# aynik/carta1

Measured on AMD Instinct MI355X. Metric: atrac1_stereo_frames_per_s_encode, higher is better.
Workload: dtype f32+f64

## Files before the change

### carta1_amd/csrc/c1_k_spec.hip

```cpp
#include "c1_device.h"

namespace {

constexpr int kR2 = 840;
constexpr int kMemFloats = kR2 + 576;
constexpr int kIn2 = 1;
struct alignas(16) SpecLds {
  alignas(16) float mem[kMemFloats];
  alignas(16) float d1[48];
  alignas(16) float d2[48];
  alignas(16) float pre2[76];
  alignas(4) uint8_t sfi[64];
  uint32_t geo[3][64];
};
constexpr int kSpecWaves = 4;
constexpr int kSpecTabBase = (int)offsetof(C1DevTables, win32);
constexpr int kSpecTabFloats = ((int)offsetof(C1DevTables, r2d) + (int)sizeof(((C1DevTables *)nullptr)->r2d) - kSpecTabBase) / 4;
static_assert(offsetof(C1DevTables, pre32_64) > offsetof(C1DevTables, win32) && offsetof(C1DevTables, r2d) > offsetof(C1DevTables, r4c) &&
              offsetof(C1DevTables, norm32) == offsetof(C1DevTables, r2d) + sizeof(((C1DevTables *)nullptr)->r2d), "win32 .. r2d are one contiguous block");
static_assert(kSpecWaves * sizeof(SpecLds) + kSpecTabFloats * 4 + 27 * 16 <= 32768, "speculative analysis: 5 workgroups of 4 waves per CU");
constexpr int kE2 = 0, kH2 = 288, kE0 = kR2, kH0 = kR2 + 160, kE1 = kR2 + 288, kH1 = kR2 + 448;

__device__ __forceinline__ int w1_phys(int v) { return __mul24(12, v >> 3) + (v & 7); }

template <int D, int NP>
__device__ __forceinline__ void qmf_core_f32(const v2f (&W)[NP], TablesPtr T, float (&lo)[D], float (&hi)[D]) {
  v2f tp[26];
#pragma unroll
  for (int j = 0; j < 26; j++) tp[j] = *reinterpret_cast<const __attribute__((address_space(4))) v2f *>(T->tap_pair[j]);
  const float e12 = T->tap32[12];
#pragma unroll
  for (int d = 0; d < D; d++) {
    v2f p1 = W[d + 23] * tp[0];
#pragma unroll
    for (int j = 1; j <= 10; j++) p1 = pk_fma(W[d + 23 - j], tp[j], p1);
    v2f p2 = W[d] * tp[23];
#pragma unroll
    for (int j = 22; j >= 13; j--) p2 = pk_fma(W[d + 23 - j], tp[j], p2);
    p1 = pk_fma(W[d + 12], tp[24], p1);
    p2 = pk_fma(W[d + 11], tp[25], p2);
    const v2f sum = p1 + p2;
    const float ev = __builtin_fmaf(e12, W[d + 11].y, sum.y);
    const float od = __builtin_fmaf(e12, W[d + 12].x, sum.x);
    lo[d] = ev + od;
    hi[d] = ev - od;
  }
}

struct SpecBase {
  int ia0, ic0;
  int q2;
  int ib, id;
  int pt0;
  int za, zb, zc, zd;
  int g;
  int e0, e1;
  int po0;
  bool band0, band2, use_lo, use_hi;
};
__device__ __forceinline__ SpecBase spec_base(int lane) {
  SpecBase B;
  const int band = lane < 16 ? 0 : (lane < 32 ? 1 : 2);
  const int g = lane - (band == 0 ? 0 : (band == 1 ? 16 : 32));
  const int n4 = band == 2 ? 128 : 64, q = n4 / 4;
  const int r = bitrev(g, band == 2 ? 5 : 4);
  const int in_base = band == 0 ? kR2 : (band == 1 ? kR2 + 256 : kIn2);
  const int tab_base = band == 2 ? (int)offsetof(C1DevTables, pre32_512) : (int)offsetof(C1DevTables, pre32_256);
  B.ia0 = in_base + 3 * n4 - 1 - 2 * r;
  B.ic0 = in_base + n4 + 2 * r;
  B.q2 = 2 * q;
  B.use_lo = r < 8;
  B.use_hi = r >= q - 8;
  B.ib = B.use_lo ? in_base + 3 * n4 + 2 * r : in_base + 2 * r + 2 * q;
  B.id = B.use_lo ? in_base + n4 - 1 - 2 * r : in_base + 14 * q - 1 - 2 * r;
  B.pt0 = tab_base + 8 * r;
  const int pbase = band == 0 ? 0 : (band == 1 ? 64 : 128);
  B.za = zslot(pbase + 4 * g);
  B.zb = zslot(pbase + 16 * (g >> 2) + (g & 3));
  B.zc = zslot(pbase + 64 * (g >> 4) + (g & 15));
  B.zd = zslot(128 + (g & 31));
  B.g = g;
  const int cbase = band == 0 ? 0 : (band == 1 ? 128 : 256), n2 = 2 * n4;
  B.e0 = cbase + 2 * g;
  B.e1 = cbase + n2 - 1 - 2 * g;
  B.po0 = tab_base + 8 * g;
  B.band0 = band == 0;
  B.band2 = band == 2;
  return B;
}

__device__ __forceinline__ void radix4_round(v2f (&x)[4], v2f wa, v2f wb, v2f wab) {
  const v2f y1 = cmul32(x[1], wa), y2 = cmul32(x[2], wb), y3 = cmul32(x[3], wab);
  const v2f t0 = x[0] + y1, t1 = x[0] - y1, t2 = y2 + y3, t3 = y2 - y3;
  x[0] = t0 + t2;
  x[2] = t0 - t2;
  x[1] = pk_fma(t3.yx, PMN, t1);
  x[3] = pk_fma(t3.yx, PNM, t1);
}

__device__ __attribute__((noinline)) bool spec_should_defer(const uint8_t *sfi, int lane, float e0, float e1, float e2,
                                                  const C1DevEncOpts *O, float threshold) {
  const int s = lane < 52 ? (int)sfi[lane] : 0;
  const float size = (float)(lane < 4 ? 8 : lane < 8 ? 4 : lane < 12 ? 8 : lane < 24 ? 6 : lane < 28 ? 7 : lane < 32 ? 9 : lane < 36 ? 10 : lane < 44 ? 12 : 20);
  const bool act = s > 0;
  const float sf = (float)s;
  const float l = __builtin_fmaf(sf, 0.33333334f, -21.0f);
  const float lb = __builtin_fmaf(O->la_slope, sf, O->la_off);
  const float eb = lane >= 36 ? e2 : (lane >= 20 ? e1 : e0);
  const float sz = act ? size : 0.0f;
  constexpr float kBudget = 1136.0f;
  const float n_all = wave_sum(sz);
  if (!(n_all > 0.0f)) return false;
  float Lw = (wave_sum(sz * lb) - kBudget) * __builtin_amdgcn_rcpf(n_all);
  {
    const float d = lb - Lw;
    const float bits = fminf(fmaxf(d, 0.0f), 16.0f);
    const float spend = wave_sum(sz * bits);
    const float n = wave_sum((d > 0.0f && d < 16.0f) ? sz : 0.0f);
    if (n > 0.0f) Lw += (spend - kBudget) * __builtin_amdgcn_rcpf(n);
  }
  const float bits = fminf(fmaxf(lb - Lw, 0.0f), 16.0f);
  const float inv_sf = __builtin_amdgcn_exp2f(-l);
  const float pm = (act && bits >= 1.0f) ? size * eb * inv_sf * __builtin_amdgcn_exp2f(bits) : 0.0f;
  const float ps = act ? fminf(1.0f, 9.7f * eb * inv_sf) : 0.0f;
  const float P = wave_sum(pm + ps);
  return !(P <= threshold);
}

__device__ __forceinline__ uint32_t spread_block(uint32_t b, uint32_t n, int bits) {
  if (bits < 4) return b;
  const uint32_t mask = (1u << bits) - 1u;
  const int sh = (bits >> 1) + 1;
  uint32_t x = b;
  do {
    x = (x * 0x9E3779B1u) & mask;
    x ^= x >> sh;
    x = (x * 0x85EBCA6Bu) & mask;
    x ^= x >> sh;
  } while (x >= n);
  return x;
}

template <bool SHORT>
__global__ __launch_bounds__(C1_WAVE * kSpecWaves, 5) void k_analysis_spec(C1EncodeLaunch L) {
  __shared__ SpecLds Sw[kSpecWaves];
  __shared__ alignas(16) float tab[kSpecTabFloats];
  __shared__ alignas(16) float tail_w[27][4];
  const int wave = __builtin_amdgcn_readfirstlane((int)(threadIdx.x >> 6));
  SpecLds &S = Sw[wave];
  const int lane0 = threadIdx.x & 63;
  int lane = lane0;
  {
    const float *src = reinterpret_cast<const float *>(reinterpret_cast<const char *>(L.tables) + kSpecTabBase);
    for (int i = threadIdx.x; i < kSpecTabFloats; i += C1_WAVE * kSpecWaves) tab[i] = src[i];
    if (threadIdx.x < 27 * 4) {
      const int idx = threadIdx.x >> 2, j = threadIdx.x & 3;
      const bool input = idx < 9;
      const int k = 4 * (input ? idx : idx - 9) - 1 + j;
      tail_w[idx][j] = (k >= 0 && k < 32) ? src[input ? 31 - k : k] : 1.0f;
    }
  }
  __syncthreads();
  const float *win = tab;
  auto table_f2 = [&](int , int byte_offset) -> v2f {
    return *reinterpret_cast<const v2f *>(reinterpret_cast<const char *>(tab) + (byte_offset - kSpecTabBase));
  };
  const uint32_t n_slots = (uint32_t)((L.frames + L.run_frames - 1) / L.run_frames) * (uint32_t)L.channels;
  const uint32_t group = L.spread_bits > 0 ? spread_block(blockIdx.x, gridDim.x, L.spread_bits) : blockIdx.x;
  const uint32_t slot = group * kSpecWaves + (uint32_t)wave;
  if (slot >= n_slots) return;
  const int ch = (int)(slot % (uint32_t)L.channels);
  const int64_t f0 = (int64_t)(slot / (uint32_t)L.channels) * L.run_frames;
  const float *__restrict__ pcm = L.pcm[ch];
  float *mem = S.mem;

  for (int i = lane; i < 48; i += 64) { S.d1[i] = 0.0f; S.d2[i] = 0.0f; }
  float ov0a = 0.0f, ov0b = 0.0f, ov1a = 0.0f, ov1b = 0.0f;
  for (int i = lane; i < 76; i += 64) S.pre2[i] = 0.0f;
  if (lane < 16) reinterpret_cast<uint32_t *>(S.sfi)[lane] = 0u;
  SpecBase B0 = spec_base(lane0);
  const SfLong SFL0 = SHORT ? sf_geometry(lane0, 2, 2, 3) : sf_long_geometry(lane0);
  if constexpr (!SHORT) {
    S.geo[0][lane0] = (uint32_t)(SFL0.src & ~3) | ((uint32_t)SFL0.b << 9) | (SFL0.wide ? 1u << 15 : 0u) | (SFL0.store ? 1u << 16 : 0u);
    S.geo[1][lane0] = (uint32_t)(B0.band0 ? B0.e0 : B0.e1) | ((uint32_t)(B0.band0 ? B0.e1 : B0.e0) << 16);
    S.geo[2][lane0] = (uint32_t)B0.po0;
  }
  if (SHORT && lane == 0) S.sfi[52] = (uint8_t)((L.opts->modes[0] & 3) | ((L.opts->modes[1] & 3) << 2) | ((L.opts->modes[2] & 3) << 4));
  const int s_band = lane0 < 16 ? 0 : (lane0 < 32 ? 1 : 2);
  const int s_g = lane0 - (s_band == 0 ? 0 : (s_band == 1 ? 16 : 32));
  const int s_blk = s_g >> 2, s_r2 = 2 * bitrev(s_g & 3, 2);
  const int s_eb0 = (s_band == 0 ? kE0 : (s_band == 1 ? kE1 : kE2)) + 32 * s_blk;
  const int s_hb0 = (s_band == 0 ? kH0 : (s_band == 1 ? kH1 : kH2)) + 32 * s_blk;
  const int s_c0 = (s_band == 0 ? 0 : (s_band == 1 ? 128 : 256)) + 32 * s_blk + 2 * (s_g & 3);
  constexpr int RT = 0;
  float p_prev = 0.0f, q_prev = 0.0f;
  wave_fence();

  const int64_t f_end = (f0 + L.run_frames < L.frames) ? f0 + L.run_frames : L.frames;
  int64_t f_first = f0 - 1;
  if (f_first < -(int64_t)L.halo_frames) f_first = -(int64_t)L.halo_frames;
  if (f_first > f0) f_first = f0;
  typedef float v4f __attribute__((ext_vector_type(4)));
  v4f pre_a, pre_b;
  {
    const v4f *p4 = reinterpret_cast<const v4f *>(pcm + f_first * 512);
    pre_a = p4[lane0]; pre_b = p4[64 + lane0];
    asm volatile("" : "+v"(pre_a), "+v"(pre_b));
  }
  uint32_t deferred_from = 0xffffffffu;
  unsigned long long open_bits = 0ull;
  for (int64_t f = f_first; f < f_end; ++f) {
    const bool emit = (f >= f0);
    TablesPtr T = tables_for_this_frame(L.tables);
    lane = lane_for_this_frame(lane0);
    if constexpr (!SHORT) {
      asm volatile("" : "+v"(B0.ia0), "+v"(B0.ic0), "+v"(B0.q2), "+v"(B0.ib), "+v"(B0.id), "+v"(B0.pt0));
      asm volatile("" : "+v"(B0.za), "+v"(B0.zb), "+v"(B0.zc), "+v"(B0.zd), "+v"(B0.g));
    }

    float P;
    {
      const v4f a = pre_a, b = pre_b;
      {
        const float pz = dpp_read<0x138>(a.z), pw = dpp_read<0x138>(a.w);
        const float qz0 = dpp_read<0x138>(b.z), qw0 = dpp_read<0x138>(b.w);
        const float az63 = lane_value(a.z, 63), aw63 = lane_value(a.w, 63);
        const float qz = lane == 0 ? az63 : qz0, qw = lane == 0 ? aw63 : qw0;
        const int v = 44 + 4 * lane;
        *reinterpret_cast<float4 *>(&mem[w1_phys(v)]) = make_float4(pz, pw, a.x, a.y);
        *reinterpret_cast<float4 *>(&mem[w1_phys(v + 256)]) = make_float4(qz, qw, b.x, b.y);
        if (lane == 63) *reinterpret_cast<float2 *>(&mem[w1_phys(556)]) = make_float2(b.z, b.w);
        if (lane < 46) mem[w1_phys(lane)] = S.d1[lane];
      }
      v2f p2 = V2(a.x, a.y) * V2(a.x, a.y);
      p2 = pk_fma(V2(a.z, a.w), V2(a.z, a.w), p2);
      p2 = pk_fma(V2(b.x, b.y), V2(b.x, b.y), p2);
      p2 = pk_fma(V2(b.z, b.w), V2(b.z, b.w), p2);
      const float p = p2.x + p2.y;
      P = wave_sum(p);
    }
    wave_fence();
    float Q;
    {
      float lo[4], hi[4];
      if (own_block()) {
        v2f W[28];
        const float4 *src = reinterpret_cast<const float4 *>(mem + __mul24(12, lane));
#pragma unroll
        for (int k = 0; k < 14; k++) {
          const float4 t = src[3 * (k >> 1) + (k & 1)];
          W[2 * k] = V2(t.x, t.y); W[2 * k + 1] = V2(t.z, t.w);
        }
        qmf_core_f32<4>(W, T, lo, hi);
      } else { for (int d = 0; d < 4; d++) { lo[d] = mem[lane + d]; hi[d] = 1.0f; } }
      {
        const v4f *p4 = reinterpret_cast<const v4f *>(pcm + ((f + 1 < f_end) ? f + 1 : f) * 512);
        pre_a = p4[lane]; pre_b = p4[64 + lane];
      }
      if (lane < 46) { S.d1[lane] = mem[w1_phys(512 + lane)]; mem[kR2 + lane] = S.d2[lane]; }
      *reinterpret_cast<float2 *>(&mem[kR2 + 46 + 4 * lane]) = make_float2(lo[0], lo[1]);
      *reinterpret_cast<float2 *>(&mem[kR2 + 48 + 4 * lane]) = make_float2(lo[2], lo[3]);
      v2f q2 = V2(lo[0], lo[1]) * V2(lo[0], lo[1]);
      q2 = pk_fma(V2(lo[2], lo[3]), V2(lo[2], lo[3]), q2);
      const float q = q2.x + q2.y;
      Q = wave_sum(q);
      if constexpr (!SHORT) {
      if (emit) for (int i = lane; i < 71; i += 64) mem[kIn2 + 112 + i] = S.pre2[1 + i];
      if (lane <= 45) {
        if (emit) *reinterpret_cast<float4 *>(&mem[kIn2 + 183 + 4 * lane]) = make_float4(hi[0], hi[1], hi[2], hi[3]);
      } else {
        const float4 wl = *reinterpret_cast<const float4 *>(tail_w[9 + lane - 46]);
        const v2f l01 = V2(hi[0], hi[1]) * V2(wl.x, wl.y), l23 = V2(hi[2], hi[3]) * V2(wl.z, wl.w);
        *reinterpret_cast<float4 *>(&S.pre2[4 * (lane - 46)]) = make_float4(l01.x, l01.y, l23.x, l23.y);
        if (lane <= 54) {
          const float4 wh = *reinterpret_cast<const float4 *>(tail_w[lane - 46]);
          const v2f h01 = V2(hi[0], hi[1]) * V2(wh.x, wh.y), h23 = V2(hi[2], hi[3]) * V2(wh.z, wh.w);
          if (emit) *reinterpret_cast<float4 *>(&mem[kIn2 + 183 + 4 * lane]) = make_float4(h01.x, h01.y, h23.x, h23.y);
        }
      }
      } else {
        if (emit) {
          if (lane < 32) mem[kE2 + lane] = S.pre2[1 + lane];
          if (lane < 39) {
            const float x = S.pre2[33 + lane];
            mem[kE2 + 32 + lane] = win[lane & 31] * x;
            mem[kH2 + lane] = x * win[31 - (lane & 31)];
          }
        }
#pragma unroll
        for (int d = 0; d < 4; d++) {
          const int pos = 39 + 4 * lane + d;
          const float x = hi[d];
          if (pos < 256) {
            const float e = win[pos & 31] * x;
            if (emit) { mem[kE2 + 32 + pos] = e; mem[kH2 + pos] = x * win[31 - (pos & 31)]; }
            if (pos >= 224) S.pre2[1 + pos - 224] = e;
          } else S.pre2[33 + pos - 256] = x;
        }
      }
    }
    wave_fence();
    {
      float lo[2], hi[2];
      if (own_block()) {
        v2f W[26];
        const float4 *src = reinterpret_cast<const float4 *>(mem + kR2 + 4 * lane);
#pragma unroll
        for (int k = 0; k < 13; k++) {
          const float4 t = src[k];
          W[2 * k] = V2(t.x, t.y); W[2 * k + 1] = V2(t.z, t.w);
        }
        qmf_core_f32<2>(W, T, lo, hi);
      } else { for (int d = 0; d < 2; d++) { lo[d] = mem[lane + d]; hi[d] = 1.0f; } }
      {
        const int ld = lane_for_this_frame(lane0);
        if (ld < 46) S.d2[ld] = mem[kR2 + 256 + ld];
      }
      if constexpr (!SHORT) {
      if (lane < 48) {
        if (emit) {
          *reinterpret_cast<float2 *>(&mem[kR2 + 80 + 2 * lane]) = make_float2(lo[0], lo[1]);
          *reinterpret_cast<float2 *>(&mem[kR2 + 256 + 80 + 2 * lane]) = make_float2(hi[0], hi[1]);
        }
      } else {
        const int k = 2 * (lane - 48);
        const float wl0 = win[k], wl1 = win[k + 1], wh0 = win[31 - k], wh1 = win[30 - k];
        if (emit) {
          *reinterpret_cast<float2 *>(&mem[kR2 + 48 + k]) = make_float2(ov0a, ov0b);
          *reinterpret_cast<float2 *>(&mem[kR2 + 256 + 48 + k]) = make_float2(ov1a, ov1b);
          *reinterpret_cast<float2 *>(&mem[kR2 + 80 + 2 * lane]) = make_float2(lo[0] * wh0, lo[1] * wh1);
          *reinterpret_cast<float2 *>(&mem[kR2 + 256 + 80 + 2 * lane]) = make_float2(hi[0] * wh0, hi[1] * wh1);
        }
        ov0a = wl0 * lo[0]; ov0b = wl1 * lo[1];
        ov1a = wl0 * hi[0]; ov1b = wl1 * hi[1];
      }
      } else {
        const int k = (2 * lane) & 31;
        const float wl0 = win[k], wl1 = win[k + 1], wh0 = win[31 - k], wh1 = win[30 - k];
        const float e00 = wl0 * lo[0], e01 = wl1 * lo[1], e10 = wl0 * hi[0], e11 = wl1 * hi[1];
        if (emit) {
          if (lane >= 48) {
            *reinterpret_cast<float2 *>(&mem[kE0 + 2 * (lane - 48)]) = make_float2(ov0a, ov0b);
            *reinterpret_cast<float2 *>(&mem[kE1 + 2 * (lane - 48)]) = make_float2(ov1a, ov1b);
          }
          *reinterpret_cast<float2 *>(&mem[kE0 + 32 + 2 * lane]) = make_float2(e00, e01);
          *reinterpret_cast<float2 *>(&mem[kE1 + 32 + 2 * lane]) = make_float2(e10, e11);
          *reinterpret_cast<float2 *>(&mem[kH0 + 2 * lane]) = make_float2(lo[0] * wh0, lo[1] * wh1);
          *reinterpret_cast<float2 *>(&mem[kH1 + 2 * lane]) = make_float2(hi[0] * wh0, hi[1] * wh1);
        }
        if (lane >= 48) { ov0a = e00; ov0b = e01; ov1a = e10; ov1b = e11; }
      }
    }
    const float W = __builtin_amdgcn_sqrtf(P + p_prev), Lw = __builtin_amdgcn_sqrtf(Q + q_prev);
    p_prev = P; q_prev = Q;
    wave_fence();
    if (!emit) {
      asm volatile("" : "+v"(pre_a), "+v"(pre_b));
      continue;
    }

    v2f x[4];
    float zrow;
    if constexpr (!SHORT) {
    const SpecBase &B = B0;
    {
      const int qb = 4 * B.q2;
      const v2f t0 = table_f2(RT, B.pt0), t1 = table_f2(RT, B.pt0 + 2 * qb);
      const v2f t2 = table_f2(RT, B.pt0 + qb), t3 = table_f2(RT, B.pt0 + __mul24(3, qb));
      const float a0 = mem[B.ia0], c0 = mem[B.ic0];
      const float a1 = mem[B.ia0 - 2 * B.q2], c1 = mem[B.ic0 + 2 * B.q2];
      const float a2 = mem[B.ia0 - B.q2], c2 = mem[B.ic0 + B.q2];
      const int q3 = __mul24(3, B.q2);
      const float a3 = mem[B.ia0 - q3], c3 = mem[B.ic0 + q3];
      const float bb = mem[B.ib], dd = mem[B.id];
      const float b0 = B.use_lo ? bb : 0.0f, d0 = B.use_lo ? dd : 0.0f;
      const float b3 = B.use_hi ? bb : 0.0f, d3 = B.use_hi ? dd : 0.0f;
      const v2f rm0 = pk_fma(V2(b0, d0), PMN, V2(a0, c0)), rm3 = pk_fma(V2(b3, d3), PNM, V2(a3, c3));
      const v2f rm1 = V2(a1, c1), rm2 = V2(a2, c2);
      auto twiddle = [](v2f rm, v2f t) { const v2f u = rm.yx * (t.yy * PMN); return pk_fma(rm, t.xx, u); };
      x[0] = twiddle(rm0, t0); x[1] = twiddle(rm1, t1); x[2] = twiddle(rm2, t2); x[3] = twiddle(rm3, t3);
      v2f en2 = x[0] * x[0];
#pragma unroll
      for (int j = 1; j < 4; j++) en2 = pk_fma(x[j], x[j], en2);
      zrow = row_allreduce(en2.x + en2.y);
      const v2f u0 = x[0] + x[1], u1 = x[0] - x[1], u2 = x[2] + x[3], u3 = x[2] - x[3];
      x[0] = u0 + u2;
      x[2] = u0 - u2;
      x[1] = pk_fma(u3.yx, PMN, u1);
      x[3] = pk_fma(u3.yx, PNM, u1);
    }
    v2f *z = reinterpret_cast<v2f *>(mem);
    {
      float4 *dst = reinterpret_cast<float4 *>(z + B.za);
      dst[0] = make_float4(x[0].x, x[0].y, x[1].x, x[1].y);
      dst[1] = make_float4(x[2].x, x[2].y, x[3].x, x[3].y);
    }
    const int twb = (int)offsetof(C1DevTables, r4b) + 24 * (B.g & 3);
    const v2f wBa = table_f2(RT, twb), wBb = table_f2(RT, twb + 8), wBc = table_f2(RT, twb + 16);
    wave_fence();
    {
      v2f *p = z + B.zb;
      x[0] = p[0]; x[1] = p[4]; x[2] = p[8]; x[3] = p[12];
      radix4_round(x, wBa, wBb, wBc);
      p[0] = x[0]; p[4] = x[1]; p[8] = x[2]; p[12] = x[3];
    }
    const int twc = (int)offsetof(C1DevTables, r4c) + 24 * (B.g & 15), twd = (int)offsetof(C1DevTables, r2d) + 8 * (B.g & 31);
    const v2f wCa = table_f2(RT, twc), wCb = table_f2(RT, twc + 8), wCc = table_f2(RT, twc + 16);
    const v2f wDa = table_f2(RT, twd), wDb = table_f2(RT, twd + 256);
    wave_fence();
    {
      v2f *p = z + B.zc;
      x[0] = p[0]; x[1] = p[20]; x[2] = p[40]; x[3] = p[60];
      radix4_round(x, wCa, wCb, wCc);
      if (B.band2) { p[0] = x[0]; p[20] = x[1]; p[40] = x[2]; p[60] = x[3]; }
    }
    const int d1 = B.band2 ? 64 : 16, d2 = 32, d3 = B.band2 ? 96 : 48;
    const int po0 = (int)S.geo[2][lane];
    const uint32_t ew = S.geo[1][lane];
    const v2f p0 = table_f2(RT, po0), p1 = table_f2(RT, po0 + 8 * d1);
    const v2f p2 = table_f2(RT, po0 + 8 * d2), p3 = table_f2(RT, po0 + 8 * d3);
    wave_fence();
    if (B.band2) {
      const v2f *p = z + B.zd;
      x[0] = p[0]; x[1] = p[80]; x[2] = p[40]; x[3] = p[120];
      const v2f y1 = cmul32(x[1], wDa), y3 = cmul32(x[3], wDb);
      const v2f e0 = x[0], e2 = x[2];
      x[0] = e0 + y1; x[1] = e0 - y1; x[2] = e2 + y3; x[3] = e2 - y3;
    }
    float *coefw = mem + kR2;
#pragma unroll
    for (int j = 0; j < 4; j++) {
      const v2f t = j == 0 ? p0 : (j == 1 ? p1 : (j == 2 ? p2 : p3));
      const int dj = j == 0 ? 0 : (j == 1 ? d1 : (j == 2 ? d2 : d3));
      const int step = B.band0 ? 2 * dj : -2 * dj;
      const v2f u = x[j].yx * (t.yy * PMN);
      const v2f o = pk_fma(x[j], t.xx, u);
      coefw[(int)(ew & 0xffffu) + step] = -o.x;
      coefw[(int)(ew >> 16) - step] = o.y;
    }
    wave_fence();

    }
    float *coef = mem + kR2;
    if constexpr (SHORT) {
    int eb = s_eb0, hb = s_hb0, r2 = s_r2;
    asm volatile("" : "+v"(eb), "+v"(hb), "+v"(r2));
    {
      const int pt = (int)offsetof(C1DevTables, pre32_64) + 4 * r2;
      const v2f t0 = table_f2(RT, pt), t1 = table_f2(RT, pt + 64), t2 = table_f2(RT, pt + 32), t3 = table_f2(RT, pt + 96);
      const float a0 = mem[hb + 15 - r2], b0 = mem[hb + 16 + r2], c0 = mem[eb + 16 + r2], d0 = mem[eb + 15 - r2];
      const float a2 = mem[hb + 7 - r2], b2 = mem[hb + 24 + r2], c2 = mem[eb + 24 + r2], d2 = mem[eb + 7 - r2];
      const float a1 = mem[eb + 31 - r2], b1 = mem[eb + r2], c1 = mem[hb + r2], d1 = mem[hb + 31 - r2];
      const float a3 = mem[eb + 23 - r2], b3 = mem[eb + 8 + r2], c3 = mem[hb + 8 + r2], d3 = mem[hb + 23 - r2];
      const v2f rm0 = pk_fma(V2(b0, d0), PMN, V2(a0, c0)), rm2 = pk_fma(V2(b2, d2), PMN, V2(a2, c2));
      const v2f rm1 = pk_fma(V2(b1, d1), PNM, V2(a1, c1)), rm3 = pk_fma(V2(b3, d3), PNM, V2(a3, c3));
      auto twiddle = [](v2f rm, v2f t) { const v2f u = rm.yx * (t.yy * PMN); return pk_fma(rm, t.xx, u); };
      x[0] = twiddle(rm0, t0); x[1] = twiddle(rm1, t1); x[2] = twiddle(rm2, t2); x[3] = twiddle(rm3, t3);
      v2f en2 = x[0] * x[0];
#pragma unroll
      for (int j = 1; j < 4; j++) en2 = pk_fma(x[j], x[j], en2);
      float en = en2.x + en2.y;
      en += dpp_read<0xB1>(en);
      en += dpp_read<0x4E>(en);
      en = fmaxf(en, dpp_read<0x141>(en));
      zrow = fmaxf(en, dpp_read<0x140>(en));
      const v2f u0 = x[0] + x[1], u1 = x[0] - x[1], u2 = x[2] + x[3], u3 = x[2] - x[3];
      x[0] = u0 + u2;
      x[2] = u0 - u2;
      x[1] = pk_fma(u3.yx, PMN, u1);
      x[3] = pk_fma(u3.yx, PNM, u1);
    }
    {
      v2f *z = reinterpret_cast<v2f *>(mem);
      int za = B0.za, zb = B0.zb, g3 = s_g & 3;
      asm volatile("" : "+v"(za), "+v"(zb), "+v"(g3));
      const int twb = (int)offsetof(C1DevTables, r4b) + 24 * g3;
      const v2f wBa = table_f2(RT, twb), wBb = table_f2(RT, twb + 8), wBc = table_f2(RT, twb + 16);
      const int po = (int)offsetof(C1DevTables, pre32_64) + 8 * g3;
      const v2f p0 = table_f2(RT, po), p1 = table_f2(RT, po + 32), p2 = table_f2(RT, po + 64), p3 = table_f2(RT, po + 96);
      wave_fence();
      float4 *dst = reinterpret_cast<float4 *>(z + za);
      dst[0] = make_float4(x[0].x, x[0].y, x[1].x, x[1].y);
      dst[1] = make_float4(x[2].x, x[2].y, x[3].x, x[3].y);
      wave_fence();
      const v2f *p = z + zb;
      x[0] = p[0]; x[1] = p[4]; x[2] = p[8]; x[3] = p[12];
      radix4_round(x, wBa, wBb, wBc);
      wave_fence();
      float *coefw = mem + kR2;
      int c0i = s_c0;
      asm volatile("" : "+v"(c0i));
      const bool band0 = B0.band0;
#pragma unroll
      for (int j = 0; j < 4; j++) {
        const v2f t = j == 0 ? p0 : (j == 1 ? p1 : (j == 2 ? p2 : p3));
        const int e0 = c0i + 8 * j, e1 = (c0i | 31) - ((c0i & 31) + 8 * j);
        const v2f u = x[j].yx * (t.yy * PMN);
        const v2f o = pk_fma(x[j], t.xx, u);
        coefw[band0 ? e0 : e1] = -o.x;
        coefw[band0 ? e1 : e0] = o.y;
      }
    }
    wave_fence();

    }
    const int64_t unit = f * L.channels + ch;
    asm volatile("" : "+v"(pre_a), "+v"(pre_b));
    {
      v4f *dst = reinterpret_cast<v4f *>(L.coefs + (unit << 9));
      const v4f *src = reinterpret_cast<const v4f *>(coef);
      const int lq = lane_for_this_frame(lane0);
      __builtin_nontemporal_store(src[lq], &dst[lq]);
      __builtin_nontemporal_store(src[64 + lq], &dst[64 + lq]);
    }
    const float Z0 = __builtin_amdgcn_sqrtf(lane_value(zrow, 0)), Z1 = __builtin_amdgcn_sqrtf(lane_value(zrow, 16));
    const float Z2 = __builtin_amdgcn_sqrtf(SHORT ? fmaxf(lane_value(zrow, 32), lane_value(zrow, 48)) : lane_value(zrow, 32) + lane_value(zrow, 48));
    const float eabs = T->spec_eabs;
    const float cz0 = SHORT ? T->spec_cz_short[0] : T->spec_cz[0], cz1 = SHORT ? T->spec_cz_short[1] : T->spec_cz[1], cz2 = SHORT ? T->spec_cz_short[2] : T->spec_cz[2];
    const float cw0 = SHORT ? T->spec_cw_short[0] : T->spec_cw[0], cw1 = SHORT ? T->spec_cw_short[1] : T->spec_cw[1], cw2 = SHORT ? T->spec_cw_short[2] : T->spec_cw[2];
    const float cl0 = SHORT ? T->spec_cl_short[0] : T->spec_cl[0], cl1 = SHORT ? T->spec_cl_short[1] : T->spec_cl[1], cl2 = SHORT ? T->spec_cl_short[2] : T->spec_cl[2];
    const float e0 = __builtin_fmaf(cz0, Z0, __builtin_fmaf(cw0, W, __builtin_fmaf(cl0, Lw, eabs)));
    const float e1 = __builtin_fmaf(cz1, Z1, __builtin_fmaf(cw1, W, __builtin_fmaf(cl1, Lw, eabs)));
    const float e2 = __builtin_fmaf(cz2, Z2, __builtin_fmaf(cw2, W, __builtin_fmaf(cl2, Lw, eabs)));
    bool unstable;
    {
      SfLong SFL = SFL0;
      float mx = 0.0f;
      if constexpr (SHORT) {
        asm volatile("" : "+v"(SFL.src), "+v"(SFL.cnt));
        const float *src = coef + SFL.src;
#pragma unroll
        for (int j = 0; j < 12; j++) mx = fmaxf(mx, fabsf(src[j < SFL.cnt ? j : SFL.cnt - 1]));
      } else {
        const uint32_t sw = S.geo[0][lane];
        SFL.b = (int)((sw >> 9) & 63u);
        SFL.wide = ((sw >> 15) & 1u) != 0u;
        SFL.store = ((sw >> 16) & 1u) != 0u;
        const float4 *grp = reinterpret_cast<const float4 *>(coef + (sw & 0x1ffu));
        mx = sf_scan_long_groups(grp[0], grp[1], grp[2]);
      }
      const float other = __int_as_float(__builtin_amdgcn_update_dpp(0, __float_as_int(mx), 0xB1, 0xf, 0xf, false));
      mx = fmaxf(mx, SFL.wide ? other : 0.0f);
      const float e = SFL.b >= 36 ? e2 : (SFL.b >= 20 ? e1 : e0);
      const float lo = fmaxf((mx - e) * 0.99999976f, 0.0f), hi = (mx + e) * 1.00000024f;
      const int s_lo = scale_factor_index_fast(lo, T->sf_m1, T->sf_m2), s_hi = scale_factor_index_fast(hi, T->sf_m1, T->sf_m2);
      if (SFL.store) S.sfi[SFL.b] = (uint8_t)s_lo;
      unstable = lane < 60 && !(s_lo == s_hi && e < __builtin_huge_valf());
    }
    const bool any_unstable = __builtin_amdgcn_ballot_w64(unstable) != 0;
    wave_fence();
    if (L.defer_list != nullptr && (((int)(f - f0)) & (kSpecCheckFrames - 1)) == 0) {
      if (spec_should_defer(S.sfi, lane, e0, e1, e2, L.opts, L.spec_defer)) { deferred_from = (uint32_t)unit; break; }
    }
    if (any_unstable) open_bits |= 1ull << (int)((f - f0) & 63);
    if (lane < 16) reinterpret_cast<uint32_t *>(L.side + unit * kSideBytes)[lane] = reinterpret_cast<const uint32_t *>(S.sfi)[lane];
    if (lane == 0) *reinterpret_cast<float4 *>(L.eps + unit * kEpsFloats) = make_float4(e0, e1, e2, __int_as_float(any_unstable ? 1 : 0));
    wave_fence();
  }
  if (L.defer_list != nullptr && lane0 == 0) L.defer_list[slot] = deferred_from;
  if (L.open_masks != nullptr && lane0 == 0) L.open_masks[slot] = open_bits;
}

__global__ __launch_bounds__(256) void k_defer_compact(const uint32_t *__restrict__ slots, uint32_t n_slots, uint32_t *__restrict__ list, uint32_t *__restrict__ counts,
                                                        int channels, int run_frames, uint32_t frames) {
  const uint32_t i = blockIdx.x * 256u + threadIdx.x;
  const uint32_t u = i < n_slots ? slots[i] : 0xffffffffu;
  const bool on = u != 0xffffffffu;
  uint32_t covered = 0;
  if (on) {
    const uint32_t f = u / (uint32_t)channels;
    uint32_t end = (f / (uint32_t)run_frames + 1u) * (uint32_t)run_frames;
    if (end > frames) end = frames;
    covered = end - f;
  }
  const uint64_t mask = __builtin_amdgcn_ballot_w64(on);
  if (mask == 0) return;
  int cov = (int)covered;
  cov = wave_inclusive_scan(cov);
  const int lane = threadIdx.x & 63;
  uint32_t at = 0;
  if (lane == 63) {
    at = atomicAdd(counts, (uint32_t)__popcll(mask));
    atomicAdd(counts + 1, (uint32_t)cov);
  }
  at = (uint32_t)__builtin_amdgcn_readlane((int)at, 63);
  if (on) list[at + __popcll(mask & ((1ull << lane) - 1ull))] = u;
}

__global__ __launch_bounds__(256) void k_open_compact(const unsigned long long *__restrict__ masks, uint32_t n_slots, uint32_t *__restrict__ list,
                                                       uint32_t *__restrict__ count, int channels, int run_frames) {
  const uint32_t i = blockIdx.x * 256u + threadIdx.x;
  unsigned long long m = i < n_slots ? masks[i] : 0ull;
  const int mine = __popcll(m);
  if (__builtin_amdgcn_ballot_w64(mine != 0) == 0) return;
  const int scan = wave_inclusive_scan(mine);
  const int lane = threadIdx.x & 63;
  uint32_t at = 0;
  if (lane == 63) at = atomicAdd(count, (uint32_t)scan);
  at = (uint32_t)__builtin_amdgcn_readlane((int)at, 63) + (uint32_t)(scan - mine);
  const uint32_t run = i / (uint32_t)channels, ch = i % (uint32_t)channels;
  while (m != 0ull) {
    const int k = __ffsll((long long)m) - 1;
    m &= m - 1ull;
    list[at++] = (run * (uint32_t)run_frames + (uint32_t)k) * (uint32_t)channels + ch;
  }
}

__global__ void k_spec_totals(unsigned long long *totals, unsigned long long units, const uint32_t *counts, int kind) {
  if (kind == 0) {
    const unsigned long long deferred = counts[4];
    totals[0] += units - deferred;
    totals[1] += counts[2] + counts[5];
    totals[2] += deferred;
    totals[3] += counts[0] - counts[2];
    totals[6] += deferred;
  } else if (kind == 1) {
    totals[2] += units;
    totals[3] += counts[0];
  } else {
    totals[4] += units;
    totals[5] += counts[0];
  }
}

}

void c1k_launch_spec_totals(unsigned long long *totals, uint64_t units, const uint32_t *counts, int kind, hipStream_t stream) {
  hipLaunchKernelGGL(k_spec_totals, dim3(1), dim3(1), 0, stream, totals, (unsigned long long)units, counts, kind);
}
void c1k_launch_open_compact(const C1EncodeLaunch &L, uint32_t *list, uint32_t *count, hipStream_t stream) {
  const int run = c1k_pick_run(L.frames, L.channels, 0);
  const int64_t slots = (L.frames + run - 1) / run * L.channels;
  hipLaunchKernelGGL(k_open_compact, dim3((unsigned)((slots + 255) / 256)), dim3(256), 0, stream, (const unsigned long long *)L.open_masks, (uint32_t)slots, list, count,
                     L.channels, run);
}
void c1k_launch_defer_compact(const C1EncodeLaunch &L, uint32_t *list, uint32_t *counts, hipStream_t stream) {
  const int run = c1k_pick_run(L.frames, L.channels, 0);
  const int64_t slots = (L.frames + run - 1) / run * L.channels;
  hipLaunchKernelGGL(k_defer_compact, dim3((unsigned)((slots + 255) / 256)), dim3(256), 0, stream, (const uint32_t *)L.defer_list, (uint32_t)slots, list, counts,
                     L.channels, run, (uint32_t)L.frames);
}

void c1k_launch_analysis_spec(const C1EncodeLaunch &L0, bool all_short, hipStream_t stream) {
  static const int slots = c1k_wave_slots(k_analysis_spec<false>);
  C1EncodeLaunch L = L0;
  L.run_frames = c1k_pick_run(L.frames, L.channels, slots);
  const int64_t runs = (L.frames + L.run_frames - 1) / L.run_frames, n_slots = runs * L.channels;
  const dim3 grid((unsigned)((n_slots + kSpecWaves - 1) / kSpecWaves)), block(C1_WAVE * kSpecWaves);
  static const bool no_spread = getenv("C1_NO_SPREAD") != nullptr;
  L.spread_bits = 0;
  if (!no_spread) while ((1ll << L.spread_bits) < (int64_t)grid.x) L.spread_bits++;
  if (all_short) hipLaunchKernelGGL((k_analysis_spec<true>), grid, block, 0, stream, L);
  else hipLaunchKernelGGL((k_analysis_spec<false>), grid, block, 0, stream, L);
}
```

Before: 190.8 million.

## Restructure spectral-analysis LDS layout and share per-lane geometry across waves

Reorganizes the per-wave LDS buffers so the QMF delay lines live inside the main mem array with a swizzled in01 layout, removing the separate d1/d2 carry buffers and their copy passes. Per-lane geometry is precomputed once per workgroup into a shared uint4 table rather than per-wave arrays, and output windows are stored in a new LDS table so the band outputs are written with uniform code. It also adds inline-asm packed multiplies with op_sel/neg modifiers for the complex twiddles, and volatile LDS loads. The aim is fewer LDS copies, fewer divergent branches and fewer VALU ops, at the cost of more intricate indexing and a reworked LDS budget check that could affect occupancy.

New measurement: 198.5 million, median of 6. 1.04x the previous value.

```diff
diff --git a/carta1_amd/csrc/c1_k_spec.hip b/carta1_amd/csrc/c1_k_spec.hip
--- a/carta1_amd/csrc/c1_k_spec.hip
+++ b/carta1_amd/csrc/c1_k_spec.hip
@@ -3,52 +3,57 @@
 namespace {
 
 constexpr int kR2 = 840;
-constexpr int kMemFloats = kR2 + 576;
+constexpr int kW2 = kR2 + 320;
+constexpr int kMemFloats = kW2 + 304;
+constexpr int kW1Tail = 768;
 constexpr int kIn2 = 1;
 struct alignas(16) SpecLds {
   alignas(16) float mem[kMemFloats];
-  alignas(16) float d1[48];
-  alignas(16) float d2[48];
   alignas(16) float pre2[76];
   alignas(4) uint8_t sfi[64];
-  uint32_t geo[3][64];
 };
+typedef uint4 SpecGeo;
+static_assert(sizeof(SpecLds) % 16 == 0 && (kW2 + 48) % 4 == 0, "16-byte groups of every wave's buffers stay aligned");
+__host__ __device__ constexpr int in01(int b, int i) { return kR2 + 64 * (i >> 5) + 32 * b + ((i & 31) ^ b); }
+
 constexpr int kSpecWaves = 4;
 constexpr int kSpecTabBase = (int)offsetof(C1DevTables, win32);
 constexpr int kSpecTabFloats = ((int)offsetof(C1DevTables, r2d) + (int)sizeof(((C1DevTables *)nullptr)->r2d) - kSpecTabBase) / 4;
 static_assert(offsetof(C1DevTables, pre32_64) > offsetof(C1DevTables, win32) && offsetof(C1DevTables, r2d) > offsetof(C1DevTables, r4c) &&
               offsetof(C1DevTables, norm32) == offsetof(C1DevTables, r2d) + sizeof(((C1DevTables *)nullptr)->r2d), "win32 .. r2d are one contiguous block");
-static_assert(kSpecWaves * sizeof(SpecLds) + kSpecTabFloats * 4 + 27 * 16 <= 32768, "speculative analysis: 5 workgroups of 4 waves per CU");
+constexpr int kSpecLdsBytes = kSpecWaves * (int)sizeof(SpecLds) + 64 * (int)sizeof(SpecGeo) + kSpecTabFloats * 4 + 28 * 16 + 64 * 8;
+static_assert((kSpecLdsBytes + 1279) / 1280 <= 25, "speculative analysis: 5 workgroups of 4 waves per CU = at most 25 LDS blocks of 1 280 bytes each");
 constexpr int kE2 = 0, kH2 = 288, kE0 = kR2, kH0 = kR2 + 160, kE1 = kR2 + 288, kH1 = kR2 + 448;
 
 __device__ __forceinline__ int w1_phys(int v) { return __mul24(12, v >> 3) + (v & 7); }
 
-template <int D, int NP>
-__device__ __forceinline__ void qmf_core_f32(const v2f (&W)[NP], TablesPtr T, float (&lo)[D], float (&hi)[D]) {
+template <int D, int NP, int OFF>
+__device__ __forceinline__ void qmf_core_f32(const v2f (&Wr)[NP], TablesPtr T, float (&lo)[D], float (&hi)[D]) {
+  static_assert(OFF + D - 1 + 23 < NP, "the window registers cover every tap");
   v2f tp[26];
 #pragma unroll
   for (int j = 0; j < 26; j++) tp[j] = *reinterpret_cast<const __attribute__((address_space(4))) v2f *>(T->tap_pair[j]);
   const float e12 = T->tap32[12];
 #pragma unroll
   for (int d = 0; d < D; d++) {
-    v2f p1 = W[d + 23] * tp[0];
-#pragma unroll
-    for (int j = 1; j <= 10; j++) p1 = pk_fma(W[d + 23 - j], tp[j], p1);
-    v2f p2 = W[d] * tp[23];
-#pragma unroll
-    for (int j = 22; j >= 13; j--) p2 = pk_fma(W[d + 23 - j], tp[j], p2);
-    p1 = pk_fma(W[d + 12], tp[24], p1);
-    p2 = pk_fma(W[d + 11], tp[25], p2);
+    v2f p1 = Wr[OFF + d + 23] * tp[0];
+#pragma unroll
+    for (int j = 1; j <= 10; j++) p1 = pk_fma(Wr[OFF + d + 23 - j], tp[j], p1);
+    v2f p2 = Wr[OFF + d] * tp[23];
+#pragma unroll
+    for (int j = 22; j >= 13; j--) p2 = pk_fma(Wr[OFF + d + 23 - j], tp[j], p2);
+    p1 = pk_fma(Wr[OFF + d + 12], tp[24], p1);
+    p2 = pk_fma(Wr[OFF + d + 11], tp[25], p2);
     const v2f sum = p1 + p2;
-    const float ev = __builtin_fmaf(e12, W[d + 11].y, sum.y);
-    const float od = __builtin_fmaf(e12, W[d + 12].x, sum.x);
+    const float ev = __builtin_fmaf(e12, Wr[OFF + d + 11].y, sum.y);
+    const float od = __builtin_fmaf(e12, Wr[OFF + d + 12].x, sum.x);
     lo[d] = ev + od;
     hi[d] = ev - od;
   }
 }
 
 struct SpecBase {
-  int ia0, ic0;
+  int ia3, ic0;
   int q2;
   int ib, id;
   int pt0;
@@ -56,6 +61,7 @@
   int g;
   int e0, e1;
   int po0;
+  int d1;
   bool band0, band2, use_lo, use_hi;
 };
 __device__ __forceinline__ SpecBase spec_base(int lane) {
@@ -64,15 +70,15 @@
   const int g = lane - (band == 0 ? 0 : (band == 1 ? 16 : 32));
   const int n4 = band == 2 ? 128 : 64, q = n4 / 4;
   const int r = bitrev(g, band == 2 ? 5 : 4);
-  const int in_base = band == 0 ? kR2 : (band == 1 ? kR2 + 256 : kIn2);
+  auto in = [band](int i) { return band == 2 ? kIn2 + i : in01(band, i); };
   const int tab_base = band == 2 ? (int)offsetof(C1DevTables, pre32_512) : (int)offsetof(C1DevTables, pre32_256);
-  B.ia0 = in_base + 3 * n4 - 1 - 2 * r;
-  B.ic0 = in_base + n4 + 2 * r;
+  B.ia3 = in(3 * n4 - 1 - 2 * r) - 192;
+  B.ic0 = in(n4 + 2 * r);
   B.q2 = 2 * q;
   B.use_lo = r < 8;
   B.use_hi = r >= q - 8;
-  B.ib = B.use_lo ? in_base + 3 * n4 + 2 * r : in_base + 2 * r + 2 * q;
-  B.id = B.use_lo ? in_base + n4 - 1 - 2 * r : in_base + 14 * q - 1 - 2 * r;
+  B.ib = B.use_lo ? in(3 * n4 + 2 * r) : in(2 * r + 2 * q);
+  B.id = B.use_lo ? in(n4 - 1 - 2 * r) : in(14 * q - 1 - 2 * r);
   B.pt0 = tab_base + 8 * r;
   const int pbase = band == 0 ? 0 : (band == 1 ? 64 : 128);
   B.za = zslot(pbase + 4 * g);
@@ -84,13 +90,29 @@
   B.e0 = cbase + 2 * g;
   B.e1 = cbase + n2 - 1 - 2 * g;
   B.po0 = tab_base + 8 * g;
+  B.d1 = band == 2 ? 64 : 16;
   B.band0 = band == 0;
   B.band2 = band == 2;
   return B;
 }
 
+__device__ __forceinline__ v2f pk_mul_yy_nyx(v2f x, v2f w) {
+  v2f r;
+  asm("v_pk_mul_f32 %0, %1, %2 op_sel:[1,1] op_sel_hi:[1,0] neg_lo:[0,1]" : "=v"(r) : "v"(x), "v"(w));
+  return r;
+}
+__device__ __forceinline__ v2f pk_mul_yx_yny(v2f x, v2f t) {
+  v2f r;
+  asm("v_pk_mul_f32 %0, %1, %2 op_sel:[1,1] op_sel_hi:[0,1] neg_hi:[0,1]" : "=v"(r) : "v"(x), "v"(t));
+  return r;
+}
+__device__ __forceinline__ v2f cmul32n(v2f x, v2f w) {
+  const v2f t = pk_mul_yy_nyx(x, w);
+  return pk_fma(x.xx, w, t);
+}
+__device__ __forceinline__ v2f lds_f2(const v2f *p) { return *(const volatile __attribute__((address_space(3))) v2f *)p; }
 __device__ __forceinline__ void radix4_round(v2f (&x)[4], v2f wa, v2f wb, v2f wab) {
-  const v2f y1 = cmul32(x[1], wa), y2 = cmul32(x[2], wb), y3 = cmul32(x[3], wab);
+  const v2f y1 = cmul32n(x[1], wa), y2 = cmul32n(x[2], wb), y3 = cmul32n(x[3], wab);
   const v2f t0 = x[0] + y1, t1 = x[0] - y1, t2 = y2 + y3, t3 = y2 - y3;
   x[0] = t0 + t2;
   x[2] = t0 - t2;
@@ -145,7 +167,9 @@
 __global__ __launch_bounds__(C1_WAVE * kSpecWaves, 5) void k_analysis_spec(C1EncodeLaunch L) {
   __shared__ SpecLds Sw[kSpecWaves];
   __shared__ alignas(16) float tab[kSpecTabFloats];
-  __shared__ alignas(16) float tail_w[27][4];
+  __shared__ alignas(16) float tail_w[28][4];
+  __shared__ alignas(8) float out_w[64][2];
+  __shared__ alignas(16) SpecGeo geo[64];
   const int wave = __builtin_amdgcn_readfirstlane((int)(threadIdx.x >> 6));
   SpecLds &S = Sw[wave];
   const int lane0 = threadIdx.x & 63;
@@ -153,17 +177,31 @@
   {
     const float *src = reinterpret_cast<const float *>(reinterpret_cast<const char *>(L.tables) + kSpecTabBase);
     for (int i = threadIdx.x; i < kSpecTabFloats; i += C1_WAVE * kSpecWaves) tab[i] = src[i];
-    if (threadIdx.x < 27 * 4) {
+    if (threadIdx.x < 28 * 4) {
       const int idx = threadIdx.x >> 2, j = threadIdx.x & 3;
-      const bool input = idx < 9;
-      const int k = 4 * (input ? idx : idx - 9) - 1 + j;
+      const bool input = idx < 10;
+      const int k = 4 * (input ? idx - 1 : idx - 10) - 1 + j;
       tail_w[idx][j] = (k >= 0 && k < 32) ? src[input ? 31 - k : k] : 1.0f;
+    }
+    if (threadIdx.x >= 128 && threadIdx.x < 128 + 64) {
+      const int l = threadIdx.x - 128, k = 2 * (l - 48);
+      out_w[l][0] = l >= 48 ? src[31 - k] : 1.0f;
+      out_w[l][1] = l >= 48 ? src[30 - k] : 1.0f;
+    }
+    if (!SHORT && threadIdx.x >= 192) {
+      const int l = threadIdx.x - 192;
+      const SpecBase G = spec_base(l);
+      const SfLong F = sf_long_geometry(l);
+      const int po = G.po0 - kSpecTabBase, u = G.band0 ? 8 * G.d1 : -8 * G.d1, t = G.band0 ? 256 : -256;
+      geo[l] = make_uint4((uint32_t)(4 * (G.band0 ? G.e0 : G.e1)) | ((uint32_t)(4 * (G.band0 ? G.e1 : G.e0)) << 16),
+                          (uint32_t)po | ((uint32_t)(po + 8 * G.d1) << 16), ((uint32_t)u & 0xffffu) | ((uint32_t)t << 16),
+                          (uint32_t)(F.src & ~3) | ((uint32_t)F.b << 9) | (F.wide ? 1u << 15 : 0u) | (F.store ? 1u << 16 : 0u));
     }
   }
   __syncthreads();
   const float *win = tab;
   auto table_f2 = [&](int , int byte_offset) -> v2f {
-    return *reinterpret_cast<const v2f *>(reinterpret_cast<const char *>(tab) + (byte_offset - kSpecTabBase));
+    return lds_f2(reinterpret_cast<const v2f *>(reinterpret_cast<const char *>(tab) + (byte_offset - kSpecTabBase)));
   };
   const uint32_t n_slots = (uint32_t)((L.frames + L.run_frames - 1) / L.run_frames) * (uint32_t)L.channels;
   const uint32_t group = L.spread_bits > 0 ? spread_block(blockIdx.x, gridDim.x, L.spread_bits) : blockIdx.x;
@@ -174,17 +212,13 @@
   const float *__restrict__ pcm = L.pcm[ch];
   float *mem = S.mem;
 
-  for (int i = lane; i < 48; i += 64) { S.d1[i] = 0.0f; S.d2[i] = 0.0f; }
+  for (int i = lane; i < 72; i += 64) mem[kW1Tail + i] = 0.0f;
+  if (lane < 48) mem[kW2 + 256 + lane] = 0.0f;
   float ov0a = 0.0f, ov0b = 0.0f, ov1a = 0.0f, ov1b = 0.0f;
   for (int i = lane; i < 76; i += 64) S.pre2[i] = 0.0f;
   if (lane < 16) reinterpret_cast<uint32_t *>(S.sfi)[lane] = 0u;
   SpecBase B0 = spec_base(lane0);
   const SfLong SFL0 = SHORT ? sf_geometry(lane0, 2, 2, 3) : sf_long_geometry(lane0);
-  if constexpr (!SHORT) {
-    S.geo[0][lane0] = (uint32_t)(SFL0.src & ~3) | ((uint32_t)SFL0.b << 9) | (SFL0.wide ? 1u << 15 : 0u) | (SFL0.store ? 1u << 16 : 0u);
-    S.geo[1][lane0] = (uint32_t)(B0.band0 ? B0.e0 : B0.e1) | ((uint32_t)(B0.band0 ? B0.e1 : B0.e0) << 16);
-    S.geo[2][lane0] = (uint32_t)B0.po0;
-  }
   if (SHORT && lane == 0) S.sfi[52] = (uint8_t)((L.opts->modes[0] & 3) | ((L.opts->modes[1] & 3) << 2) | ((L.opts->modes[2] & 3) << 4));
   const int s_band = lane0 < 16 ? 0 : (lane0 < 32 ? 1 : 2);
   const int s_g = lane0 - (s_band == 0 ? 0 : (s_band == 1 ? 16 : 32));
@@ -214,7 +248,7 @@
     TablesPtr T = tables_for_this_frame(L.tables);
     lane = lane_for_this_frame(lane0);
     if constexpr (!SHORT) {
-      asm volatile("" : "+v"(B0.ia0), "+v"(B0.ic0), "+v"(B0.q2), "+v"(B0.ib), "+v"(B0.id), "+v"(B0.pt0));
+      asm volatile("" : "+v"(B0.ia3), "+v"(B0.ic0), "+v"(B0.q2), "+v"(B0.ib), "+v"(B0.id), "+v"(B0.pt0));
       asm volatile("" : "+v"(B0.za), "+v"(B0.zb), "+v"(B0.zc), "+v"(B0.zd), "+v"(B0.g));
     }
 
@@ -222,15 +256,13 @@
     {
       const v4f a = pre_a, b = pre_b;
       {
-        const float pz = dpp_read<0x138>(a.z), pw = dpp_read<0x138>(a.w);
-        const float qz0 = dpp_read<0x138>(b.z), qw0 = dpp_read<0x138>(b.w);
-        const float az63 = lane_value(a.z, 63), aw63 = lane_value(a.w, 63);
-        const float qz = lane == 0 ? az63 : qz0, qw = lane == 0 ? aw63 : qw0;
-        const int v = 44 + 4 * lane;
-        *reinterpret_cast<float4 *>(&mem[w1_phys(v)]) = make_float4(pz, pw, a.x, a.y);
-        *reinterpret_cast<float4 *>(&mem[w1_phys(v + 256)]) = make_float4(qz, qw, b.x, b.y);
-        if (lane == 63) *reinterpret_cast<float2 *>(&mem[w1_phys(556)]) = make_float2(b.z, b.w);
-        if (lane < 46) mem[w1_phys(lane)] = S.d1[lane];
+        const int p = w1_phys(lane);
+        float dl = 0.0f;
+        if (lane < 48) dl = mem[kW1Tail + p];
+        const int s = __mul24(6, lane) - 2 * (lane & 1);
+        *reinterpret_cast<v4f *>(&mem[72 + s]) = a;
+        *reinterpret_cast<v4f *>(&mem[72 + 384 + s]) = b;
+        if (lane < 48) mem[p] = dl;
       }
       v2f p2 = V2(a.x, a.y) * V2(a.x, a.y);
       p2 = pk_fma(V2(a.z, a.w), V2(a.z, a.w), p2);
@@ -248,35 +280,34 @@
         const float4 *src = reinterpret_cast<const float4 *>(mem + __mul24(12, lane));
 #pragma unroll
         for (int k = 0; k < 14; k++) {
-          const float4 t = src[3 * (k >> 1) + (k & 1)];
+          v4f t = *reinterpret_cast<const v4f *>(&src[3 * (k >> 1) + (k & 1)]);
+          if (k == 0) asm volatile("" : "+v"(t));
           W[2 * k] = V2(t.x, t.y); W[2 * k + 1] = V2(t.z, t.w);
         }
-        qmf_core_f32<4>(W, T, lo, hi);
+        qmf_core_f32<4, 28, 1>(W, T, lo, hi);
       } else { for (int d = 0; d < 4; d++) { lo[d] = mem[lane + d]; hi[d] = 1.0f; } }
       {
         const v4f *p4 = reinterpret_cast<const v4f *>(pcm + ((f + 1 < f_end) ? f + 1 : f) * 512);
         pre_a = p4[lane]; pre_b = p4[64 + lane];
       }
-      if (lane < 46) { S.d1[lane] = mem[w1_phys(512 + lane)]; mem[kR2 + lane] = S.d2[lane]; }
-      *reinterpret_cast<float2 *>(&mem[kR2 + 46 + 4 * lane]) = make_float2(lo[0], lo[1]);
-      *reinterpret_cast<float2 *>(&mem[kR2 + 48 + 4 * lane]) = make_float2(lo[2], lo[3]);
+      if (lane < 48) mem[kW2 + lane] = mem[kW2 + 256 + lane];
+      *reinterpret_cast<float4 *>(&mem[kW2 + 48 + 4 * lane]) = make_float4(lo[0], lo[1], lo[2], lo[3]);
       v2f q2 = V2(lo[0], lo[1]) * V2(lo[0], lo[1]);
       q2 = pk_fma(V2(lo[2], lo[3]), V2(lo[2], lo[3]), q2);
       const float q = q2.x + q2.y;
       Q = wave_sum(q);
       if constexpr (!SHORT) {
-      if (emit) for (int i = lane; i < 71; i += 64) mem[kIn2 + 112 + i] = S.pre2[1 + i];
-      if (lane <= 45) {
-        if (emit) *reinterpret_cast<float4 *>(&mem[kIn2 + 183 + 4 * lane]) = make_float4(hi[0], hi[1], hi[2], hi[3]);
-      } else {
-        const float4 wl = *reinterpret_cast<const float4 *>(tail_w[9 + lane - 46]);
+      if (emit && lane < 36) *reinterpret_cast<float2 *>(&mem[kIn2 + 111 + 2 * lane]) = *reinterpret_cast<const float2 *>(&S.pre2[2 * lane]);
+      {
+        const int wi = min(max(lane - 45, 0), 10);
+        const float4 wh = *reinterpret_cast<const float4 *>(tail_w[wi]);
+        const v2f h01 = V2(hi[0], hi[1]) * V2(wh.x, wh.y), h23 = V2(hi[2], hi[3]) * V2(wh.z, wh.w);
+        if (emit && lane <= 54) *reinterpret_cast<float4 *>(&mem[kIn2 + 183 + 4 * lane]) = make_float4(h01.x, h01.y, h23.x, h23.y);
+      }
+      if (lane >= 46) {
+        const float4 wl = *reinterpret_cast<const float4 *>(tail_w[10 + lane - 46]);
         const v2f l01 = V2(hi[0], hi[1]) * V2(wl.x, wl.y), l23 = V2(hi[2], hi[3]) * V2(wl.z, wl.w);
         *reinterpret_cast<float4 *>(&S.pre2[4 * (lane - 46)]) = make_float4(l01.x, l01.y, l23.x, l23.y);
-        if (lane <= 54) {
-          const float4 wh = *reinterpret_cast<const float4 *>(tail_w[lane - 46]);
-          const v2f h01 = V2(hi[0], hi[1]) * V2(wh.x, wh.y), h23 = V2(hi[2], hi[3]) * V2(wh.z, wh.w);
-          if (emit) *reinterpret_cast<float4 *>(&mem[kIn2 + 183 + 4 * lane]) = make_float4(h01.x, h01.y, h23.x, h23.y);
-        }
       }
       } else {
         if (emit) {
@@ -304,32 +335,32 @@
       float lo[2], hi[2];
       if (own_block()) {
         v2f W[26];
-        const float4 *src = reinterpret_cast<const float4 *>(mem + kR2 + 4 * lane);
+        const float4 *src = reinterpret_cast<const float4 *>(mem + kW2 + 4 * lane);
 #pragma unroll
         for (int k = 0; k < 13; k++) {
-          const float4 t = src[k];
+          v4f t = *reinterpret_cast<const v4f *>(&src[k]);
+          if (k == 0) asm volatile("" : "+v"(t));
           W[2 * k] = V2(t.x, t.y); W[2 * k + 1] = V2(t.z, t.w);
         }
-        qmf_core_f32<2>(W, T, lo, hi);
+        qmf_core_f32<2, 26, 1>(W, T, lo, hi);
       } else { for (int d = 0; d < 2; d++) { lo[d] = mem[lane + d]; hi[d] = 1.0f; } }
+      if constexpr (!SHORT) {
+      const int u = lane + 40, at = kR2 + 2 * (u + (u & ~15));
       {
-        const int ld = lane_for_this_frame(lane0);
-        if (ld < 46) S.d2[ld] = mem[kR2 + 256 + ld];
-      }
-      if constexpr (!SHORT) {
-      if (lane < 48) {
+        const v2f wh = *reinterpret_cast<const v2f *>(out_w[lane]);
+        const v2f o0 = V2(lo[0], lo[1]) * wh, o1 = V2(hi[1], hi[0]) * wh.yx;
         if (emit) {
-          *reinterpret_cast<float2 *>(&mem[kR2 + 80 + 2 * lane]) = make_float2(lo[0], lo[1]);
-          *reinterpret_cast<float2 *>(&mem[kR2 + 256 + 80 + 2 * lane]) = make_float2(hi[0], hi[1]);
+          *reinterpret_cast<v2f *>(&mem[at]) = o0;
+          *reinterpret_cast<v2f *>(&mem[at + 32]) = o1;
         }
-      } else {
+      }
+      if (lane >= 48) {
         const int k = 2 * (lane - 48);
-        const float wl0 = win[k], wl1 = win[k + 1], wh0 = win[31 - k], wh1 = win[30 - k];
+        const float wl0 = win[k], wl1 = win[k + 1];
         if (emit) {
-          *reinterpret_cast<float2 *>(&mem[kR2 + 48 + k]) = make_float2(ov0a, ov0b);
-          *reinterpret_cast<float2 *>(&mem[kR2 + 256 + 48 + k]) = make_float2(ov1a, ov1b);
-          *reinterpret_cast<float2 *>(&mem[kR2 + 80 + 2 * lane]) = make_float2(lo[0] * wh0, lo[1] * wh1);
-          *reinterpret_cast<float2 *>(&mem[kR2 + 256 + 80 + 2 * lane]) = make_float2(hi[0] * wh0, hi[1] * wh1);
+          const int uo = lane - 24, ato = kR2 + 2 * (uo + (uo & ~15));
+          *reinterpret_cast<float2 *>(&mem[ato]) = make_float2(ov0a, ov0b);
+          *reinterpret_cast<float2 *>(&mem[ato + 32]) = make_float2(ov1b, ov1a);
         }
         ov0a = wl0 * lo[0]; ov0b = wl1 * lo[1];
         ov1a = wl0 * hi[0]; ov1b = wl1 * hi[1];
@@ -361,23 +392,23 @@
 
     v2f x[4];
     float zrow;
+    uint32_t gw_sf = 0;
     if constexpr (!SHORT) {
     const SpecBase &B = B0;
     {
       const int qb = 4 * B.q2;
       const v2f t0 = table_f2(RT, B.pt0), t1 = table_f2(RT, B.pt0 + 2 * qb);
       const v2f t2 = table_f2(RT, B.pt0 + qb), t3 = table_f2(RT, B.pt0 + __mul24(3, qb));
-      const float a0 = mem[B.ia0], c0 = mem[B.ic0];
-      const float a1 = mem[B.ia0 - 2 * B.q2], c1 = mem[B.ic0 + 2 * B.q2];
-      const float a2 = mem[B.ia0 - B.q2], c2 = mem[B.ic0 + B.q2];
-      const int q3 = __mul24(3, B.q2);
-      const float a3 = mem[B.ia0 - q3], c3 = mem[B.ic0 + q3];
+      const float a0 = mem[B.ia3 + 192], c0 = mem[B.ic0];
+      const float a1 = mem[B.ia3 + 64], c1 = mem[B.ic0 + 128];
+      const float a2 = mem[B.ia3 + 128], c2 = mem[B.ic0 + 64];
+      const float a3 = mem[B.ia3], c3 = mem[B.ic0 + 192];
       const float bb = mem[B.ib], dd = mem[B.id];
       const float b0 = B.use_lo ? bb : 0.0f, d0 = B.use_lo ? dd : 0.0f;
       const float b3 = B.use_hi ? bb : 0.0f, d3 = B.use_hi ? dd : 0.0f;
       const v2f rm0 = pk_fma(V2(b0, d0), PMN, V2(a0, c0)), rm3 = pk_fma(V2(b3, d3), PNM, V2(a3, c3));
       const v2f rm1 = V2(a1, c1), rm2 = V2(a2, c2);
-      auto twiddle = [](v2f rm, v2f t) { const v2f u = rm.yx * (t.yy * PMN); return pk_fma(rm, t.xx, u); };
+      auto twiddle = [](v2f rm, v2f t) { const v2f u = pk_mul_yx_yny(rm, t); return pk_fma(rm, t.xx, u); };
       x[0] = twiddle(rm0, t0); x[1] = twiddle(rm1, t1); x[2] = twiddle(rm2, t2); x[3] = twiddle(rm3, t3);
       v2f en2 = x[0] * x[0];
 #pragma unroll
@@ -400,7 +431,7 @@
     wave_fence();
     {
       v2f *p = z + B.zb;
-      x[0] = p[0]; x[1] = p[4]; x[2] = p[8]; x[3] = p[12];
+      x[0] = lds_f2(p); x[1] = lds_f2(p + 4); x[2] = lds_f2(p + 8); x[3] = lds_f2(p + 12);
       radix4_round(x, wBa, wBb, wBc);
       p[0] = x[0]; p[4] = x[1]; p[8] = x[2]; p[12] = x[3];
     }
@@ -410,34 +441,35 @@
     wave_fence();
     {
       v2f *p = z + B.zc;
-      x[0] = p[0]; x[1] = p[20]; x[2] = p[40]; x[3] = p[60];
+      x[0] = lds_f2(p); x[1] = lds_f2(p + 20); x[2] = lds_f2(p + 40); x[3] = lds_f2(p + 60);
       radix4_round(x, wCa, wCb, wCc);
       if (B.band2) { p[0] = x[0]; p[20] = x[1]; p[40] = x[2]; p[60] = x[3]; }
     }
-    const int d1 = B.band2 ? 64 : 16, d2 = 32, d3 = B.band2 ? 96 : 48;
-    const int po0 = (int)S.geo[2][lane];
-    const uint32_t ew = S.geo[1][lane];
-    const v2f p0 = table_f2(RT, po0), p1 = table_f2(RT, po0 + 8 * d1);
-    const v2f p2 = table_f2(RT, po0 + 8 * d2), p3 = table_f2(RT, po0 + 8 * d3);
+    const SpecGeo gw = geo[lane];
+    const int po0 = kSpecTabBase + (int)(gw.y & 0xffffu), po1 = kSpecTabBase + (int)(gw.y >> 16);
+    const v2f p0 = table_f2(RT, po0), p1 = table_f2(RT, po1);
+    const v2f p2 = table_f2(RT, po0 + 256), p3 = table_f2(RT, po1 + 256);
     wave_fence();
     if (B.band2) {
       const v2f *p = z + B.zd;
-      x[0] = p[0]; x[1] = p[80]; x[2] = p[40]; x[3] = p[120];
-      const v2f y1 = cmul32(x[1], wDa), y3 = cmul32(x[3], wDb);
+      x[0] = lds_f2(p); x[1] = lds_f2(p + 80); x[2] = lds_f2(p + 40); x[3] = lds_f2(p + 120);
+      const v2f y1 = cmul32n(x[1], wDa), y3 = cmul32n(x[3], wDb);
       const v2f e0 = x[0], e2 = x[2];
       x[0] = e0 + y1; x[1] = e0 - y1; x[2] = e2 + y3; x[3] = e2 - y3;
     }
-    float *coefw = mem + kR2;
+    char *coefw = reinterpret_cast<char *>(mem + kR2);
+    const int cf = (int)(gw.x & 0xffffu), cs = (int)(gw.x >> 16);
+    const int su = (int)(gw.z << 16) >> 16, st = (int)gw.z >> 16, sut = su + st;
 #pragma unroll
     for (int j = 0; j < 4; j++) {
       const v2f t = j == 0 ? p0 : (j == 1 ? p1 : (j == 2 ? p2 : p3));
-      const int dj = j == 0 ? 0 : (j == 1 ? d1 : (j == 2 ? d2 : d3));
-      const int step = B.band0 ? 2 * dj : -2 * dj;
-      const v2f u = x[j].yx * (t.yy * PMN);
+      const int step = j == 0 ? 0 : (j == 1 ? su : (j == 2 ? st : sut));
+      const v2f u = pk_mul_yx_yny(x[j], t);
       const v2f o = pk_fma(x[j], t.xx, u);
-      coefw[(int)(ew & 0xffffu) + step] = -o.x;
-      coefw[(int)(ew >> 16) - step] = o.y;
-    }
+      *reinterpret_cast<float *>(coefw + (cf + step)) = -o.x;
+      *reinterpret_cast<float *>(coefw + (cs - step)) = o.y;
+    }
+    gw_sf = gw.w;
     wave_fence();
 
     }
@@ -532,7 +564,7 @@
 #pragma unroll
         for (int j = 0; j < 12; j++) mx = fmaxf(mx, fabsf(src[j < SFL.cnt ? j : SFL.cnt - 1]));
       } else {
-        const uint32_t sw = S.geo[0][lane];
+        const uint32_t sw = gw_sf;
         SFL.b = (int)((sw >> 9) & 63u);
         SFL.wide = ((sw >> 15) & 1u) != 0u;
         SFL.store = ((sw >> 16) & 1u) != 0u;
```
